# GiaKhangLuu/SCFlow

Hardware: AMD Instinct MI355X
Metric: refinement iters/s (batch×GRU-steps/s) at 256×256, 1/2/4/8 MI355X (higher is better)
Workload: dtype f32; 1 GPU; SCFlowDecoder forward, 16 pairs/GPU, 256x256, 8 GRU iters (BASELINE configs[1]); global_batch=16, image=256, iters=8, launch=eager, schedule=whole batch, parallelism=dp1

## Files before the change

scflow_amd/csrc/lookup_conv.hip:

```cpp
#include "common.h"

namespace {

constexpr int LC_PX = 64;
constexpr int LC_R = 4;
constexpr int LC_D = 2 * LC_R + 1;
constexpr int LC_L = 4;
constexpr int LC_K = LC_L * LC_D * LC_D;
constexpr int LC_KB = (LC_K + 7) / 8;
constexpr int LC_KP = 8 * LC_KB + 4;
constexpr int LC_TRW = 16;
constexpr int LC_WP = LC_TRW * LC_TRW + 4;
constexpr int LC_PD = 3;
constexpr int LC_OOB = 0x7ffffff0;
constexpr int LC_KEND[LC_L] = {(1 * LC_D * LC_D) / 8, (2 * LC_D * LC_D) / 8, (3 * LC_D * LC_D) / 8,
                               LC_KB};
__host__ __device__ constexpr int lc_level(int kb) {
  return kb < LC_KEND[0] ? 0 : kb < LC_KEND[1] ? 1 : kb < LC_KEND[2] ? 2 : 3;
}

__device__ __forceinline__ __amdgpu_buffer_rsrc_t lc_rsrc(const void* p, unsigned bytes) {
  return __builtin_amdgcn_make_buffer_rsrc(const_cast<void*>(p), (short)0, (int)bytes, 0x00020000);
}
__device__ __forceinline__ floatx4 lc_bload4(__amdgpu_buffer_rsrc_t r, int voff, int soff) {
  return __builtin_bit_cast(floatx4, __builtin_amdgcn_raw_buffer_load_b128(r, voff, soff, 0));
}

__device__ __forceinline__ float lc_unnorm(float s, int size, int ac) {
#pragma clang fp contract(off)
  const float g = (s * 2.f) / (float)(size - 1 > 1 ? size - 1 : 1) - 1.f;
  return ac ? ((g + 1.f) / 2.f) * (float)(size - 1) : ((g + 1.f) * (float)size - 1.f) / 2.f;
}

struct LcArgs {
  const float* pyr;
  const float* flow;
  const float* weight;
  const float* bias;
  const float* mask;
  float* out;
  int so, n, h, w, cout, act, ac;
};

__global__ __launch_bounds__(512, 1) void corr_lookup_conv1x1_kernel(LcArgs a) {
#pragma clang fp contract(off)
  extern __shared__ floatx4 smem4[];
  float* As = (float*)smem4;
  float* Wn = As + LC_PX * LC_KP;
  const int tid = threadIdx.x, lane = tid & 63;
  const int wave = __builtin_amdgcn_readfirstlane(tid >> 6);
  const bool producer = wave >= 4;
  const int li = lane & 31, hh = lane >> 5;
  const int H = a.h, W = a.w, P = H * W;
  const long long M = (long long)a.n * P;
  const long long m0 = (long long)blockIdx.x * LC_PX;
  const int npad = (a.cout + 63) / 64 * 64;
  const bool wave_on = !producer && wave * 64 < npad;
  float bias_v[2] = {0.f, 0.f};
  if (wave_on && a.bias) {
#pragma unroll
    for (int nb = 0; nb < 2; ++nb) {
      const int col = 64 * wave + 32 * nb + li;
      if (col < a.cout) bias_v[nb] = a.bias[col];
    }
  }

  const int pt = producer ? tid - 256 : 0;
  const int ps = pt >> 2, sub = pt & 3;
  const long long gp = m0 + ps;
  const bool active = gp < M;
  const int p = active ? (int)(gp % P) : 0;
  const int y = p / W, x = p % W;
  float fx = 0.f, fy = 0.f;
  float mk = 1.f;
  if (active) {
    fx = a.flow[gp * 2];
    fy = a.flow[gp * 2 + 1];
    if (a.mask) mk = a.mask[gp];
  }
  const long long left = M - m0;
  const int npx = left < LC_PX ? (int)left : LC_PX;

  auto origin = [&](int l, int axis, float c0x, float c0y) __attribute__((always_inline)) {
    const bool fin = isfinite(c0x) && isfinite(c0y) && fabsf(c0x) < 1e8f && fabsf(c0y) < 1e8f;
    int o = fin ? (int)floorf(axis == 0 ? c0x : c0y) - 1 : -(1 << 29);
    return ((axis == 0 ? W : H) >> l) <= 8 ? -4 : (o >> 2) << 2;
  };
  auto first = [&](int l, int axis) __attribute__((always_inline)) {
    const int size = axis == 0 ? (W >> l) : (H >> l);
    const float c = ((float)(axis == 0 ? x : y) + (axis == 0 ? fx : fy)) / (float)(1 << l);
    return lc_unnorm(c + (float)(0 - LC_R), size, a.ac);
  };

  auto last = [&](int l, int axis) __attribute__((always_inline)) {
    const int size = axis == 0 ? (W >> l) : (H >> l);
    const float c = ((float)(axis == 0 ? x : y) + (axis == 0 ? fx : fy)) / (float)(1 << l);
    return lc_unnorm(c + (float)LC_R, size, a.ac);
  };

  floatx4 wr[16];
  auto rload = [&](int l) __attribute__((always_inline)) {
    size_t loff = 0;
    for (int k = 0; k < l; ++k) loff += (size_t)M * ((H >> k) * (W >> k));
    const int Hl = H >> l, Wl = W >> l, hw = Hl * Wl;
    const __amdgpu_buffer_rsrc_t rs =
        lc_rsrc(a.pyr + loff + (size_t)m0 * hw, (unsigned)(npx * hw * 4));
    const float c0x = first(l, 0), c0y = first(l, 1);
    const int ox = origin(l, 0, c0x, c0y), oy = origin(l, 1, c0x, c0y);
    const float c1x = last(l, 0), c1y = last(l, 1);
    const bool fin = isfinite(c0x) && isfinite(c0y) && fabsf(c0x) < 1e8f && fabsf(c0y) < 1e8f &&
                     isfinite(c1x) && isfinite(c1y) && fabsf(c1x) < 1e8f && fabsf(c1y) < 1e8f;
    const int xlo = fin ? (int)floorf(c0x) : 1, xhi = fin ? (int)floorf(c1x) + 1 : 0;
    const int ylo = fin ? (int)floorf(c0y) : 1, yhi = fin ? (int)floorf(c1y) + 1 : 0;
#pragma unroll
    for (int j = 0; j < 16; ++j) {
      const int k = sub + 4 * j, kt = k >> 2;
      const int gx = ox + (kt & 3) * 4, gy = oy + (kt >> 2) * 4 + (k & 3);
      const bool ok = active && gx >= 0 && gx < Wl && gy >= 0 && gy < Hl && gy >= ylo &&
                      gy <= yhi && gx + 3 >= xlo && gx <= xhi;
      const int e = ((gy >> 2) * (Wl >> 2) + (gx >> 2)) * 16 + (gy & 3) * 4;
      wr[j] = lc_bload4(rs, ok ? (ps * hw + e) * 4 : LC_OOB, 0);
    }
  };
  auto rstore = [&]() __attribute__((always_inline)) {
    float* sw = Wn + ps * LC_WP;
#pragma unroll
    for (int j = 0; j < 16; ++j) {
      const int k = sub + 4 * j, kt = k >> 2;
      *(floatx4*)(sw + ((kt >> 2) * 4 + (k & 3)) * LC_TRW + (kt & 3) * 4) = wr[j];
    }
  };
  auto sample = [&](int l) __attribute__((always_inline)) {
#pragma clang fp contract(off)
    const int Hl = H >> l, Wl = W >> l;
    const float scale = (float)(1 << l);
    const float cx = ((float)x + fx) / scale, cy = ((float)y + fy) / scale;
    const float c0x = lc_unnorm(cx + (float)(0 - LC_R), Wl, a.ac);
    const float c0y = lc_unnorm(cy + (float)(0 - LC_R), Hl, a.ac);
    const bool fin = isfinite(c0x) && isfinite(c0y) && fabsf(c0x) < 1e8f && fabsf(c0y) < 1e8f;
    const int ox = origin(l, 0, c0x, c0y), oy = origin(l, 1, c0x, c0y);
    float iy[LC_D];
    int ry[LC_D];
#pragma unroll
    for (int b = 0; b < LC_D; ++b) {
      iy[b] = lc_unnorm(cy + (float)(b - LC_R), Hl, a.ac);
      ry[b] = fin && isfinite(iy[b]) ? (int)floorf(iy[b]) - oy : -1;
    }
    const float* sw = Wn + ps * LC_WP;
    float* arow = As + ps * LC_KP + l * LC_D * LC_D;
#pragma unroll
    for (int q = 0; q < 3; ++q) {
      const int aa = sub + 4 * q;
      if (aa < LC_D) {
        const float ix = lc_unnorm(cx + (float)(aa - LC_R), Wl, a.ac);
        const int rx = fin && isfinite(ix) ? (int)floorf(ix) - ox : -1;
        const bool okx = active && rx >= 0 && rx + 1 < LC_TRW;
        float t00[LC_D], t01[LC_D], t10[LC_D], t11[LC_D];
        bool ok[LC_D];
#pragma unroll
        for (int b = 0; b < LC_D; ++b) {
          ok[b] = okx && ry[b] >= 0 && ry[b] + 1 < LC_TRW;
          const float* wp = sw + (ok[b] ? ry[b] * LC_TRW + rx : 0);
          t00[b] = wp[0];
          t01[b] = wp[1];
          t10[b] = wp[LC_TRW];
          t11[b] = wp[LC_TRW + 1];
        }
        const float ix_w = floorf(ix), ix_e = ix_w + 1.f;
        const float wxw = ix_e - ix, wxe = ix - ix_w;
#pragma unroll
        for (int b = 0; b < LC_D; ++b) {
          const float iy_n = floorf(iy[b]), iy_s = iy_n + 1.f;
          const float wyn = iy_s - iy[b], wys = iy[b] - iy_n;
          float v = 0.f;
          v += t00[b] * (wxw * wyn);
          v += t01[b] * (wxe * wyn);
          v += t10[b] * (wxw * wys);
          v += t11[b] * (wxe * wys);
          arow[aa * LC_D + b] = (ok[b] ? v : 0.f) * mk;
        }
      }
    }
  };

  const __amdgpu_buffer_rsrc_t wsrc = lc_rsrc(a.weight + (size_t)(2 * wave) * LC_KB * 256,
                                              (unsigned)(wave_on ? 2 * LC_KB * 1024 : 0));
  auto bload = [&](floatx4(&bb)[2], int kb) {
    const int k = kb < LC_KB ? kb : LC_KB - 1;
#pragma unroll
    for (int nb = 0; nb < 2; ++nb) bb[nb] = lc_bload4(wsrc, lane * 16, (nb * LC_KB + k) * 1024);
  };
  floatx16 acc[2][2];
#pragma unroll
  for (int i = 0; i < 2; ++i)
#pragma unroll
    for (int j = 0; j < 2; ++j)
#pragma unroll
      for (int e = 0; e < 16; ++e) acc[i][j][e] = 0.f;
  floatx4 bq[LC_PD][2];
  const float* ar0 = As + li * LC_KP + 4 * hh;
  const float* ar1 = As + (32 + li) * LC_KP + 4 * hh;
  floatx4 an0, an1;
  auto body = [&](auto kbc) __attribute__((always_inline)) {
    constexpr int kb = decltype(kbc)::value, sl = kb % LC_PD;
    constexpr int l = lc_level(kb);
    constexpr bool opens = kb == (l == 0 ? 0 : LC_KEND[l == 0 ? 0 : l - 1]);
    constexpr bool last = kb + 1 == LC_KEND[l];
    if constexpr (opens) {
      an0 = *(const floatx4*)(ar0 + 8 * kb);
      an1 = *(const floatx4*)(ar1 + 8 * kb);
    }
    const floatx4 a0 = an0, a1 = an1;
    floatx4 b[2] = {bq[sl][0], bq[sl][1]};
    if constexpr (kb + LC_PD < LC_KB) bload(bq[sl], kb + LC_PD);
    if constexpr (!last) {
      an0 = *(const floatx4*)(ar0 + 8 * (kb + 1));
      an1 = *(const floatx4*)(ar1 + 8 * (kb + 1));
    }
    __builtin_amdgcn_sched_barrier(0);
#pragma unroll
    for (int e = 0; e < 4; ++e) {
      acc[0][0] = __builtin_amdgcn_mfma_f32_32x32x2f32(a0[e], b[0][e], acc[0][0], 0, 0, 0);
      acc[0][1] = __builtin_amdgcn_mfma_f32_32x32x2f32(a0[e], b[1][e], acc[0][1], 0, 0, 0);
      acc[1][0] = __builtin_amdgcn_mfma_f32_32x32x2f32(a1[e], b[0][e], acc[1][0], 0, 0, 0);
      acc[1][1] = __builtin_amdgcn_mfma_f32_32x32x2f32(a1[e], b[1][e], acc[1][1], 0, 0, 0);
    }
    __builtin_amdgcn_sched_barrier(0);
  };
  auto regions_to_lds = [&]() __attribute__((always_inline)) {
    rstore();
    __builtin_amdgcn_s_waitcnt(0xc07f);
    __builtin_amdgcn_wave_barrier();
  };

  if (producer) {
    rload(0);
    regions_to_lds();
    sample(0);
  } else {
#pragma unroll
    for (int d = 0; d < LC_PD; ++d) bload(bq[d], d);
    if (tid < LC_PX) {
#pragma unroll
      for (int c = LC_K; c < 8 * LC_KB; ++c) As[tid * LC_KP + c] = 0.f;
    }
  }
  __syncthreads();
  auto phase = [&](auto lc) __attribute__((always_inline)) {
    constexpr int l = decltype(lc)::value;
    if (producer) {
      if constexpr (l < LC_L) {
        rload(l);
        regions_to_lds();
        sample(l);
      }
    } else {
      StaticFor<(l == 1 ? 0 : LC_KEND[l == 1 ? 0 : l - 2]), LC_KEND[l - 1]>::run(body);
    }
    if constexpr (l < LC_L) __syncthreads();
  };
  StaticFor<1, LC_L + 1>::run(phase);

  if (!wave_on) return;
  auto store = [&](auto actc) __attribute__((always_inline)) {
    constexpr int ACT = decltype(actc)::value;
#pragma unroll
    for (int nb = 0; nb < 2; ++nb) {
      const int col = 64 * wave + 32 * nb + li;
      if (col >= a.cout) continue;
#pragma unroll
      for (int mb = 0; mb < 2; ++mb)
#pragma unroll
        for (int r = 0; r < 16; ++r) {
          const long long m = m0 + 32 * mb + (r & 3) + 8 * (r >> 2) + 4 * hh;
          if (m < M) a.out[m * a.so + col] = act_apply(acc[mb][nb][r] + bias_v[nb], ACT);
        }
    }
  };
  switch (a.act) {
    case SCFLOW_ACT_RELU: store(std::integral_constant<int, SCFLOW_ACT_RELU>{}); break;
    case SCFLOW_ACT_SIGMOID: store(std::integral_constant<int, SCFLOW_ACT_SIGMOID>{}); break;
    case SCFLOW_ACT_TANH: store(std::integral_constant<int, SCFLOW_ACT_TANH>{}); break;
    default: store(std::integral_constant<int, SCFLOW_ACT_NONE>{}); break;
  }
}

}

SCFLOW_API long long scflow_corr_lookup_conv1x1_lds_bytes(void) {
  return (long long)sizeof(float) * LC_PX * (LC_KP + LC_WP);
}

static int lookup_conv1x1_launch(const float* pyr, const float* flow, const float* mask,
                                 const float* weight, const float* bias, float* out, int out_stride,
                                 int n, int h, int w, int num_levels, int radius, int cout, int act,
                                 int align_corners, void* stream) {
  if (!pyr || !flow || !weight || !out || n <= 0 || h <= 0 || w <= 0 || cout <= 0 ||
      out_stride < cout)
    return SCFLOW_EINVAL;
  if (num_levels != LC_L || radius != LC_R || cout > 256 || h % 32 || w % 32)
    return SCFLOW_EUNSUPPORTED;
  if (!aligned16(pyr) || !aligned16(weight)) return SCFLOW_EALIGN;
  if ((long long)LC_PX * h * w * 4 >= LC_OOB) return SCFLOW_EUNSUPPORTED;
  LcArgs a;
  a.pyr = pyr;
  a.flow = flow;
  a.weight = weight;
  a.bias = bias;
  a.mask = mask;
  a.out = out;
  a.so = out_stride;
  a.n = n;
  a.h = h;
  a.w = w;
  a.cout = cout;
  a.act = act;
  a.ac = align_corners ? 1 : 0;
  const size_t lds = (size_t)scflow_corr_lookup_conv1x1_lds_bytes();
  static bool attr = false;
  if (!attr) {
    (void)hipFuncSetAttribute((const void*)corr_lookup_conv1x1_kernel,
                              hipFuncAttributeMaxDynamicSharedMemorySize, 160 * 1024);
    attr = true;
  }
  const long long M = (long long)n * h * w;
  corr_lookup_conv1x1_kernel<<<(unsigned)((M + LC_PX - 1) / LC_PX), 512, lds, (hipStream_t)stream>>>(a);
  return scflow_launch_status();
}

SCFLOW_API int scflow_corr_lookup_conv1x1(const float* pyr, const float* flow, const float* weight,
                                          const float* bias, float* out, int out_stride, int n,
                                          int h, int w, int num_levels, int radius, int cout,
                                          int act, int align_corners, void* stream) {
  return lookup_conv1x1_launch(pyr, flow, nullptr, weight, bias, out, out_stride, n, h, w,
                               num_levels, radius, cout, act, align_corners, stream);
}

SCFLOW_API int scflow_corr_lookup_conv1x1_masked(const float* pyr, const float* flow,
                                                 const float* mask, const float* weight,
                                                 const float* bias, float* out, int out_stride,
                                                 int n, int h, int w, int num_levels, int radius,
                                                 int cout, int act, int align_corners,
                                                 void* stream) {
  return lookup_conv1x1_launch(pyr, flow, mask, weight, bias, out, out_stride, n, h, w, num_levels,
                               radius, cout, act, align_corners, stream);
}
```

Measured before the change: 28470 iters/s.

## Double producer lanes per pixel and prefetch next pyramid level during sampling

The producer side of the fused correlation-lookup plus 1x1 conv kernel now uses 8 lanes per pixel by default (8 producer waves, 768 threads). Sampling rows are split across lane halves. Per-level bilinear coordinates are computed once into a small double-buffered LDS table instead of being recomputed in every lane. The producer is restructured to issue the next level's region loads before sampling the current level, so global-load latency overlaps with sampling. This is meant to shorten the producer critical path that gates the MFMA consumer waves, at the cost of more threads, extra LDS and added barriers. Optional timestamp instrumentation is added behind a compile flag.

```diff
diff --git a/scflow_amd/csrc/lookup_conv.hip b/scflow_amd/csrc/lookup_conv.hip
--- a/scflow_amd/csrc/lookup_conv.hip
+++ b/scflow_amd/csrc/lookup_conv.hip
@@ -11,8 +11,17 @@
 constexpr int LC_KP = 8 * LC_KB + 4;
 constexpr int LC_TRW = 16;
 constexpr int LC_WP = LC_TRW * LC_TRW + 4;
+constexpr int LC_CTP = 2 * LC_D + 2;
 constexpr int LC_PD = 3;
 constexpr int LC_OOB = 0x7ffffff0;
+#ifndef LC_PL
+#define LC_PL 8
+#endif
+static_assert(LC_PL == 4 || LC_PL == 8, "producer lanes per pixel");
+constexpr int LC_PWAVES = LC_PL * LC_PX / 64;
+constexpr int LC_THREADS = 256 + 64 * LC_PWAVES;
+constexpr int LC_NR = 64 / LC_PL;
+constexpr int LC_NB = LC_PL == 8 ? 5 : LC_D;
 constexpr int LC_KEND[LC_L] = {(1 * LC_D * LC_D) / 8, (2 * LC_D * LC_D) / 8, (3 * LC_D * LC_D) / 8,
                                LC_KB};
 __host__ __device__ constexpr int lc_level(int kb) {
@@ -40,13 +49,28 @@
   const float* mask;
   float* out;
   int so, n, h, w, cout, act, ac;
+#ifdef LC_STAMPS
+  unsigned long long* stamps;
+#endif
 };
 
-__global__ __launch_bounds__(512, 1) void corr_lookup_conv1x1_kernel(LcArgs a) {
+#ifdef LC_STAMPS
+constexpr int LC_NST = 18;
+#define LC_STAMP(who, k)                                                                 \
+  do {                                                                                    \
+    if (a.stamps && threadIdx.x == (who))                                                 \
+      a.stamps[(size_t)blockIdx.x * LC_NST + (k)] = __builtin_amdgcn_s_memrealtime();     \
+  } while (0)
+#else
+#define LC_STAMP(who, k) ((void)0)
+#endif
+
+__global__ __launch_bounds__(LC_THREADS, 1) void corr_lookup_conv1x1_kernel(LcArgs a) {
 #pragma clang fp contract(off)
   extern __shared__ floatx4 smem4[];
   float* As = (float*)smem4;
   float* Wn = As + LC_PX * LC_KP;
+  float* Ct = Wn + LC_PX * LC_WP;
   const int tid = threadIdx.x, lane = tid & 63;
   const int wave = __builtin_amdgcn_readfirstlane(tid >> 6);
   const bool producer = wave >= 4;
@@ -66,7 +90,8 @@
   }
 
   const int pt = producer ? tid - 256 : 0;
-  const int ps = pt >> 2, sub = pt & 3;
+  const int ps = pt / LC_PL, pj = pt % LC_PL, sub = pj & 3;
+  const int b0 = (pj >> 2) * LC_NB;
   const long long gp = m0 + ps;
   const bool active = gp < M;
   const int p = active ? (int)(gp % P) : 0;
@@ -86,35 +111,41 @@
     int o = fin ? (int)floorf(axis == 0 ? c0x : c0y) - 1 : -(1 << 29);
     return ((axis == 0 ? W : H) >> l) <= 8 ? -4 : (o >> 2) << 2;
   };
-  auto first = [&](int l, int axis) __attribute__((always_inline)) {
-    const int size = axis == 0 ? (W >> l) : (H >> l);
-    const float c = ((float)(axis == 0 ? x : y) + (axis == 0 ? fx : fy)) / (float)(1 << l);
-    return lc_unnorm(c + (float)(0 - LC_R), size, a.ac);
-  };
-
-  auto last = [&](int l, int axis) __attribute__((always_inline)) {
-    const int size = axis == 0 ? (W >> l) : (H >> l);
-    const float c = ((float)(axis == 0 ? x : y) + (axis == 0 ? fx : fy)) / (float)(1 << l);
-    return lc_unnorm(c + (float)LC_R, size, a.ac);
-  };
-
-  floatx4 wr[16];
+  auto ctab = [&](int l) __attribute__((always_inline)) { return Ct + ((l & 1) * LC_PX + ps) * LC_CTP; };
+  auto coords = [&](int l) __attribute__((always_inline)) {
+#pragma clang fp contract(off)
+    const int Hl = H >> l, Wl = W >> l;
+    const float scale = (float)(1 << l);
+    const float cx = ((float)x + fx) / scale, cy = ((float)y + fy) / scale;
+    float* ct = ctab(l);
+#pragma unroll
+    for (int s = 0; s < (2 * LC_D + LC_PL - 1) / LC_PL; ++s) {
+      const int f = pj + LC_PL * s;
+      const bool ya = f >= LC_D;
+      const int i = ya ? f - LC_D : f;
+      const float v = lc_unnorm((ya ? cy : cx) + (float)(i - LC_R), ya ? Hl : Wl, a.ac);
+      if (f < 2 * LC_D) ct[f] = v;
+    }
+  };
+
+  floatx4 wr[LC_NR];
   auto rload = [&](int l) __attribute__((always_inline)) {
     size_t loff = 0;
     for (int k = 0; k < l; ++k) loff += (size_t)M * ((H >> k) * (W >> k));
     const int Hl = H >> l, Wl = W >> l, hw = Hl * Wl;
     const __amdgpu_buffer_rsrc_t rs =
         lc_rsrc(a.pyr + loff + (size_t)m0 * hw, (unsigned)(npx * hw * 4));
-    const float c0x = first(l, 0), c0y = first(l, 1);
+    const float* ct = ctab(l);
+    const float c0x = ct[0], c0y = ct[LC_D];
     const int ox = origin(l, 0, c0x, c0y), oy = origin(l, 1, c0x, c0y);
-    const float c1x = last(l, 0), c1y = last(l, 1);
+    const float c1x = ct[LC_D - 1], c1y = ct[2 * LC_D - 1];
     const bool fin = isfinite(c0x) && isfinite(c0y) && fabsf(c0x) < 1e8f && fabsf(c0y) < 1e8f &&
                      isfinite(c1x) && isfinite(c1y) && fabsf(c1x) < 1e8f && fabsf(c1y) < 1e8f;
     const int xlo = fin ? (int)floorf(c0x) : 1, xhi = fin ? (int)floorf(c1x) + 1 : 0;
     const int ylo = fin ? (int)floorf(c0y) : 1, yhi = fin ? (int)floorf(c1y) + 1 : 0;
 #pragma unroll
-    for (int j = 0; j < 16; ++j) {
-      const int k = sub + 4 * j, kt = k >> 2;
+    for (int j = 0; j < LC_NR; ++j) {
+      const int k = pj + LC_PL * j, kt = k >> 2;
       const int gx = ox + (kt & 3) * 4, gy = oy + (kt >> 2) * 4 + (k & 3);
       const bool ok = active && gx >= 0 && gx < Wl && gy >= 0 && gy < Hl && gy >= ylo &&
                       gy <= yhi && gx + 3 >= xlo && gx <= xhi;
@@ -125,25 +156,22 @@
   auto rstore = [&]() __attribute__((always_inline)) {
     float* sw = Wn + ps * LC_WP;
 #pragma unroll
-    for (int j = 0; j < 16; ++j) {
-      const int k = sub + 4 * j, kt = k >> 2;
+    for (int j = 0; j < LC_NR; ++j) {
+      const int k = pj + LC_PL * j, kt = k >> 2;
       *(floatx4*)(sw + ((kt >> 2) * 4 + (k & 3)) * LC_TRW + (kt & 3) * 4) = wr[j];
     }
   };
   auto sample = [&](int l) __attribute__((always_inline)) {
 #pragma clang fp contract(off)
-    const int Hl = H >> l, Wl = W >> l;
-    const float scale = (float)(1 << l);
-    const float cx = ((float)x + fx) / scale, cy = ((float)y + fy) / scale;
-    const float c0x = lc_unnorm(cx + (float)(0 - LC_R), Wl, a.ac);
-    const float c0y = lc_unnorm(cy + (float)(0 - LC_R), Hl, a.ac);
+    const float* ct = ctab(l);
+    const float c0x = ct[0], c0y = ct[LC_D];
     const bool fin = isfinite(c0x) && isfinite(c0y) && fabsf(c0x) < 1e8f && fabsf(c0y) < 1e8f;
     const int ox = origin(l, 0, c0x, c0y), oy = origin(l, 1, c0x, c0y);
-    float iy[LC_D];
-    int ry[LC_D];
-#pragma unroll
-    for (int b = 0; b < LC_D; ++b) {
-      iy[b] = lc_unnorm(cy + (float)(b - LC_R), Hl, a.ac);
+    float iy[LC_NB];
+    int ry[LC_NB];
+#pragma unroll
+    for (int b = 0; b < LC_NB; ++b) {
+      iy[b] = ct[LC_D + (b0 + b < LC_D ? b0 + b : LC_D - 1)];
       ry[b] = fin && isfinite(iy[b]) ? (int)floorf(iy[b]) - oy : -1;
     }
     const float* sw = Wn + ps * LC_WP;
@@ -152,13 +180,13 @@
     for (int q = 0; q < 3; ++q) {
       const int aa = sub + 4 * q;
       if (aa < LC_D) {
-        const float ix = lc_unnorm(cx + (float)(aa - LC_R), Wl, a.ac);
+        const float ix = ct[aa];
         const int rx = fin && isfinite(ix) ? (int)floorf(ix) - ox : -1;
         const bool okx = active && rx >= 0 && rx + 1 < LC_TRW;
-        float t00[LC_D], t01[LC_D], t10[LC_D], t11[LC_D];
-        bool ok[LC_D];
-#pragma unroll
-        for (int b = 0; b < LC_D; ++b) {
+        float t00[LC_NB], t01[LC_NB], t10[LC_NB], t11[LC_NB];
+        bool ok[LC_NB];
+#pragma unroll
+        for (int b = 0; b < LC_NB; ++b) {
           ok[b] = okx && ry[b] >= 0 && ry[b] + 1 < LC_TRW;
           const float* wp = sw + (ok[b] ? ry[b] * LC_TRW + rx : 0);
           t00[b] = wp[0];
@@ -169,7 +197,7 @@
         const float ix_w = floorf(ix), ix_e = ix_w + 1.f;
         const float wxw = ix_e - ix, wxe = ix - ix_w;
 #pragma unroll
-        for (int b = 0; b < LC_D; ++b) {
+        for (int b = 0; b < LC_NB; ++b) {
           const float iy_n = floorf(iy[b]), iy_s = iy_n + 1.f;
           const float wyn = iy_s - iy[b], wys = iy[b] - iy_n;
           float v = 0.f;
@@ -177,11 +205,50 @@
           v += t01[b] * (wxe * wyn);
           v += t10[b] * (wxw * wys);
           v += t11[b] * (wxe * wys);
-          arow[aa * LC_D + b] = (ok[b] ? v : 0.f) * mk;
+          if (b0 + b < LC_D) arow[aa * LC_D + b0 + b] = (ok[b] ? v : 0.f) * mk;
         }
       }
     }
   };
+
+  auto regions_to_lds = [&]() __attribute__((always_inline)) {
+    rstore();
+    __builtin_amdgcn_s_waitcnt(0xc07f);
+    __builtin_amdgcn_wave_barrier();
+  };
+
+  LC_STAMP(0, 0);
+  if (producer) {
+    coords(0);
+    coords(1);
+    __builtin_amdgcn_s_waitcnt(0xc07f);
+    __builtin_amdgcn_wave_barrier();
+    rload(0);
+    regions_to_lds();
+    LC_STAMP(256, 1);
+    rload(1);
+    __builtin_amdgcn_sched_barrier(0);
+    sample(0);
+    LC_STAMP(256, 5);
+    __syncthreads();
+    auto pphase = [&](auto lc) __attribute__((always_inline)) {
+      constexpr int l = decltype(lc)::value;
+      __builtin_amdgcn_s_waitcnt(0xc07f);
+      __builtin_amdgcn_wave_barrier();
+      if constexpr (l + 1 < LC_L) coords(l + 1);
+      regions_to_lds();
+      LC_STAMP(256, 1 + l);
+      if constexpr (l + 1 < LC_L) {
+        rload(l + 1);
+        __builtin_amdgcn_sched_barrier(0);
+      }
+      sample(l);
+      LC_STAMP(256, 5 + l);
+      __syncthreads();
+    };
+    StaticFor<1, LC_L>::run(pphase);
+    return;
+  }
 
   const __amdgpu_buffer_rsrc_t wsrc = lc_rsrc(a.weight + (size_t)(2 * wave) * LC_KB * 256,
                                               (unsigned)(wave_on ? 2 * LC_KB * 1024 : 0));
@@ -227,39 +294,21 @@
     }
     __builtin_amdgcn_sched_barrier(0);
   };
-  auto regions_to_lds = [&]() __attribute__((always_inline)) {
-    rstore();
-    __builtin_amdgcn_s_waitcnt(0xc07f);
-    __builtin_amdgcn_wave_barrier();
-  };
-
-  if (producer) {
-    rload(0);
-    regions_to_lds();
-    sample(0);
-  } else {
-#pragma unroll
-    for (int d = 0; d < LC_PD; ++d) bload(bq[d], d);
-    if (tid < LC_PX) {
-#pragma unroll
-      for (int c = LC_K; c < 8 * LC_KB; ++c) As[tid * LC_KP + c] = 0.f;
-    }
+#pragma unroll
+  for (int d = 0; d < LC_PD; ++d) bload(bq[d], d);
+  if (tid < LC_PX) {
+#pragma unroll
+    for (int c = LC_K; c < 8 * LC_KB; ++c) As[tid * LC_KP + c] = 0.f;
   }
   __syncthreads();
-  auto phase = [&](auto lc) __attribute__((always_inline)) {
+  auto cphase = [&](auto lc) __attribute__((always_inline)) {
     constexpr int l = decltype(lc)::value;
-    if (producer) {
-      if constexpr (l < LC_L) {
-        rload(l);
-        regions_to_lds();
-        sample(l);
-      }
-    } else {
-      StaticFor<(l == 1 ? 0 : LC_KEND[l == 1 ? 0 : l - 2]), LC_KEND[l - 1]>::run(body);
-    }
+    LC_STAMP(0, 9 + 2 * (l - 1));
+    StaticFor<(l == 1 ? 0 : LC_KEND[l == 1 ? 0 : l - 2]), LC_KEND[l - 1]>::run(body);
+    LC_STAMP(0, 10 + 2 * (l - 1));
     if constexpr (l < LC_L) __syncthreads();
   };
-  StaticFor<1, LC_L + 1>::run(phase);
+  StaticFor<1, LC_L + 1>::run(cphase);
 
   if (!wave_on) return;
   auto store = [&](auto actc) __attribute__((always_inline)) {
@@ -283,13 +332,22 @@
     case SCFLOW_ACT_TANH: store(std::integral_constant<int, SCFLOW_ACT_TANH>{}); break;
     default: store(std::integral_constant<int, SCFLOW_ACT_NONE>{}); break;
   }
+  LC_STAMP(0, 17);
 }
 
 }
 
 SCFLOW_API long long scflow_corr_lookup_conv1x1_lds_bytes(void) {
-  return (long long)sizeof(float) * LC_PX * (LC_KP + LC_WP);
-}
+  return (long long)sizeof(float) * LC_PX * (LC_KP + LC_WP + 2 * LC_CTP);
+}
+
+#ifdef LC_STAMPS
+static unsigned long long* g_lc_stamps = nullptr;
+SCFLOW_API int scflow_debug_lookup_conv_stamps(void* stamps) {
+  g_lc_stamps = (unsigned long long*)stamps;
+  return LC_NST;
+}
+#endif
 
 static int lookup_conv1x1_launch(const float* pyr, const float* flow, const float* mask,
                                  const float* weight, const float* bias, float* out, int out_stride,
@@ -316,6 +374,9 @@
   a.cout = cout;
   a.act = act;
   a.ac = align_corners ? 1 : 0;
+#ifdef LC_STAMPS
+  a.stamps = g_lc_stamps;
+#endif
   const size_t lds = (size_t)scflow_corr_lookup_conv1x1_lds_bytes();
   static bool attr = false;
   if (!attr) {
@@ -324,7 +385,7 @@
     attr = true;
   }
   const long long M = (long long)n * h * w;
-  corr_lookup_conv1x1_kernel<<<(unsigned)((M + LC_PX - 1) / LC_PX), 512, lds, (hipStream_t)stream>>>(a);
+  corr_lookup_conv1x1_kernel<<<(unsigned)((M + LC_PX - 1) / LC_PX), LC_THREADS, lds, (hipStream_t)stream>>>(a);
   return scflow_launch_status();
 }
 
```

Result: faster. 28810 iters/s, median of 6 (+1.2%).
